# DLR-RM/3DObjectTracking

Measured on NVIDIA H100. Metric: pose-opt iterations/sec (bodies x corr_iters), higher is better.
Workload: dtype f32

## Files before the change

### 3dobjecttracking_b200/csrc/m3t_b200_track2.cuh

```cuda
#pragma once

#include "m3t_b200_kernels.cuh"
#include "m3t_b200_views.cuh"

namespace m3tb {

constexpr int kGroup = 512;
constexpr int kDistBytes = kDistributionLength * kGroup * 4;
constexpr int kClusterStage = 96;
constexpr int kClusterBytes = 2 * kClusterStage * 32;
constexpr int kFixedDynBytes = kDistBytes + kClusterBytes;

struct BinImage {
  const uint16_t* px;
  unsigned pitch;
};

struct Shared2 {
  float pose[12];
  float rb2c[12], db2c[12];
  float dc2b[12];
  float cw2c[12], dw2c[12];
  float view_o[2][4];
  Tile ctile, dtile;
  unsigned long long depth_bar, lut_bar, ctile_bar;
  float red[32][32];
  float a[36], b[6], x[6];
  int views[2][2];
  FrameView cframe, dframe;
  int stamp_n[2];
  BodyDev body;
  CameraDev cams[2];
  ModelDev models[2];
  const float4* info[2];
  BinImage bins;
};

template <int T>
__device__ __forceinline__ void GroupBarrier(int group) {
  if (T == kGroup) __syncthreads();
  else asm volatile("bar.sync %0, %1;" ::"r"(group + 1), "r"(kGroup) : "memory");
}

struct LineRegs {
  float cbx, cby, cbz, cu, cv, nu, nv, dr, ncts, mean, var;
  bool valid;
};

template <int T>
__device__ __forceinline__ void Stamp2(const TrackArgs& args, Shared2& sh) {
  const int tid = threadIdx.x, warp = tid >> 5;
  if (!args.phase_clock || (tid & 31) != 0) return;
  if (warp != T / 32 - 1 && !(T > kGroup && warp == kGroup / 32 - 1)) return;
  const int half = (T > kGroup && tid < kGroup) ? 1 : 0;
  const int i = sh.stamp_n[half];
  if (i < kPhaseSlots / 2) {
    args.phase_clock[size_t(blockIdx.x) * kPhaseSlots + half * (kPhaseSlots / 2) + i] = clock64();
    sh.stamp_n[half] = i + 1;
  }
}

#define M3TB_STAMP_AT(slot, cond)                                                                  \
  do {                                                                                             \
    if (args.phase_clock && (cond)) args.phase_clock[size_t(body_id) * kPhaseSlots + (slot)] = clock64(); \
  } while (0)

template <bool LUT_SMEM, int S>
__device__ __forceinline__ void WalkFast(int scale, int base, float minor_f, float step, int stride_major, int stride_minor,
                                         const uint16_t* tile_px, const float2* __restrict__ lut_g, const float2* lut_s,
                                         const float* __restrict__ lf, const float* __restrict__ lb, bool rev,
                                         float* dist_col) {
  float wf[8], wb[8];
#pragma unroll
  for (int w = 0; w < kLineSegments; ++w) {
    float pf = 1.0f, pb = 1.0f;
    if (S > 0) {
      int idx[S > 0 ? S : 1];
#pragma unroll
      for (int k = 0; k < S; ++k) {
        idx[k] = tile_px[base + int(minor_f) * stride_minor];
        base += stride_major;
        minor_f += step;
      }
      float2 l[S > 0 ? S : 1];
#pragma unroll
      for (int k = 0; k < S; ++k) l[k] = LutFetch<LUT_SMEM>(lut_g, lut_s, idx[k]);
#pragma unroll
      for (int k = 0; k < S; ++k) { pf *= l[k].x; pb *= l[k].y; }
    } else {
#pragma unroll 1
      for (int k = 0; k < scale; ++k) {
        const int idx = tile_px[base + int(minor_f) * stride_minor];
        const float2 l = LutFetch<LUT_SMEM>(lut_g, lut_s, idx);
        pf *= l.x;
        pb *= l.y;
        base += stride_major;
        minor_f += step;
      }
    }
    if (S > 1 || (S == 0 && scale > 1)) {
      if (pf != 0.0f || pb != 0.0f) {
        float sum = pf;
        sum += pb;
        pf /= sum;
        pb /= sum;
      } else {
        pf = 0.5f;
        pb = 0.5f;
      }
    }
    wf[w & 7] = pf;
    wb[w & 7] = pb;
    if (w >= 7) {
      float val = 1.0f;
#pragma unroll
      for (int k = 0; k < kFunctionLength; ++k) {
        const float f = rev ? wf[(w - k) & 7] : wf[(w + 1 + k) & 7];
        const float b = rev ? wb[(w - k) & 7] : wb[(w + 1 + k) & 7];
        val *= f * lf[k] + b * lb[k];
      }
      dist_col[(rev ? kLineSegments - 1 - w : w - 7) * kGroup] = val;
    }
  }
}

template <bool LUT_SMEM>
__device__ __noinline__ void WalkSlow(int scale, int bs, int nb, bool horizontal, int major, float minor_f, float step,
                                      const FrameView& frame, const Tile& tile, const uint16_t* tile_px, const BinImage& bins,
                                      const float2* __restrict__ lut_g, const float2* lut_s, const float* lf,
                                      const float* lb, bool rev, float* dist_col) {
  float sf[kLineSegments], sb[kLineSegments];
#pragma unroll 1
  for (int s = 0; s < kLineSegments; ++s) {
    float pf = 1.0f, pb = 1.0f;
#pragma unroll 1
    for (int k = 0; k < scale; ++k) {
      const int minor = int(minor_f);
      const int x = horizontal ? major : minor, y = horizontal ? minor : major;
      const unsigned tx = unsigned(x - tile.x0), ty = unsigned(y - tile.y0);
      int idx;
      if (tx < unsigned(tile.w) && ty < unsigned(tile.h)) {
        idx = tile_px[ty * unsigned(tile.pitch) + tx];
      } else if (bins.px && x >= frame.x0 && x < frame.x1 && y >= frame.y0 && y < frame.y1) {
        idx = __ldg(reinterpret_cast<const uint16_t*>(reinterpret_cast<const uint8_t*>(bins.px) + size_t(unsigned(y)) * bins.pitch) + x);
      } else {
        const uint8_t* p = FramePtr(frame, x, y, 3u);
        idx = int(LutSlot(unsigned((int(__ldg(p)) >> bs) * nb * nb + (int(__ldg(p + 1)) >> bs) * nb + (int(__ldg(p + 2)) >> bs))));
      }
      const float2 l = LutFetch<LUT_SMEM>(lut_g, lut_s, idx);
      pf *= l.x;
      pb *= l.y;
      ++major;
      minor_f += step;
    }
    sf[s] = pf;
    sb[s] = pb;
  }
  if (scale > 1) {
#pragma unroll 1
    for (int s = 0; s < kLineSegments; ++s) {
      if (sf[s] != 0.0f || sb[s] != 0.0f) {
        float sum = sf[s];
        sum += sb[s];
        sf[s] /= sum;
        sb[s] /= sum;
      } else {
        sf[s] = 0.5f;
        sb[s] = 0.5f;
      }
    }
  }
#pragma unroll 1
  for (int d = 0; d < kDistributionLength; ++d) {
    float val = 1.0f;
#pragma unroll 1
    for (int k = 0; k < kFunctionLength; ++k) {
      const int s = rev ? kLineSegments - 1 - (d + k) : d + k;
      val *= sf[s] * lf[k] + sb[s] * lb[k];
    }
    dist_col[d * kGroup] = val;
  }
}

template <bool LUT_SMEM>
__device__ __forceinline__ void RegionLine2(const RegionIter& it, const RegionParamsDev& rp, const float4 p0, const float4 p1,
                                            const FrameView& frame, const Tile& tile, const uint16_t* tile_px,
                                            const BinImage& bins, const float2* __restrict__ lut_g, const float2* lut_s,
                                            const float* __restrict__ lf, const float* __restrict__ lb,
                                            float* dist_col, LineRegs& L) {
  L.valid = false;
  float x, y, z;
  PoseApply(it.b2c, p0.x, p0.y, p0.z, x, y, z);
  float nu = it.b2c[0] * p0.w + it.b2c[1] * p1.x + it.b2c[2] * p1.y;
  float nv = it.b2c[4] * p0.w + it.b2c[5] * p1.x + it.b2c[6] * p1.y;
  {
    float zz = nu * nu + nv * nv;
    if (zz > 0.0f) { float n = sqrtf(zz); nu /= n; nv /= n; }
  }
  float center_u = x * it.fu / z + it.ppu;
  float center_v = y * it.fv / z + it.ppv;
  L.cbx = p0.x; L.cby = p0.y; L.cbz = p0.z;
  L.cu = center_u; L.cv = center_v; L.nu = nu; L.nv = nv;
  float continuous_distance = fminf(p1.w, p1.z) * it.fu / (z * it.fscale);
  if (continuous_distance < rp.min_continuous_distance) return;
  if (z <= 0.0f) return;
  int icu = int(center_u + 0.5f), icv = int(center_v + 0.5f);
  if (icu < 0 || icu > it.w_m1 || icv < 0 || icv > it.h_m1) return;
  const bool horizontal = fabsf(nv) < fabsf(nu);
  const float c_major = horizontal ? center_u : center_v;
  const float c_minor = horizontal ? center_v : center_u;
  const float n_major = horizontal ? nu : nv;
  const float n_minor = horizontal ? nv : nu;
  const int major_m1 = horizontal ? it.w_m1 : it.h_m1;
  const int minor_m1 = horizontal ? it.h_m1 : it.w_m1;
  const int minor_m2 = horizontal ? it.h_m2 : it.w_m2;
  const float step = n_minor / n_major;
  int major = int(c_major - it.ll_half_m1);
  const int major_end = major + it.ll_m1;
  float minor_f = c_minor + step * (float(major) - c_major) + 0.5f;
  const float minor_f_end = minor_f + step * float(it.ll_m1);
  if (major < 0 || major_end > major_m1 || int(minor_f) < 0 || int(minor_f) > minor_m1 || int(minor_f_end) < 1 ||
      int(minor_f_end) > minor_m2)
    return;
  const bool rev = !(n_major > 0.0f);
  {
    const int mi0 = int(minor_f), mi1 = int(minor_f_end);
    const int minor_lo = min(mi0, mi1) - 1, minor_hi = max(mi0, mi1) + 1;
    const int x_lo = horizontal ? major : minor_lo, x_hi = horizontal ? major_end : minor_hi;
    const int y_lo = horizontal ? minor_lo : major, y_hi = horizontal ? minor_hi : major_end;
    const bool inside = x_lo >= tile.x0 && x_hi < tile.x0 + tile.w && y_lo >= tile.y0 && y_hi < tile.y0 + tile.h;
    if (inside) {
      const int stride_major = horizontal ? 1 : tile.pitch;
      const int stride_minor = horizontal ? tile.pitch : 1;
      const int base = horizontal ? (major - tile.x0) - tile.y0 * tile.pitch : (major - tile.y0) * tile.pitch - tile.x0;
      switch (it.scale) {
        case 1: WalkFast<LUT_SMEM, 1>(1, base, minor_f, step, stride_major, stride_minor, tile_px, lut_g, lut_s, lf, lb, rev, dist_col); break;
        case 2: WalkFast<LUT_SMEM, 2>(2, base, minor_f, step, stride_major, stride_minor, tile_px, lut_g, lut_s, lf, lb, rev, dist_col); break;
        case 4: WalkFast<LUT_SMEM, 4>(4, base, minor_f, step, stride_major, stride_minor, tile_px, lut_g, lut_s, lf, lb, rev, dist_col); break;
        case 6: WalkFast<LUT_SMEM, 6>(6, base, minor_f, step, stride_major, stride_minor, tile_px, lut_g, lut_s, lf, lb, rev, dist_col); break;
        default: WalkFast<LUT_SMEM, 0>(it.scale, base, minor_f, step, stride_major, stride_minor, tile_px, lut_g, lut_s, lf, lb, rev, dist_col); break;
      }
    } else {
      WalkSlow<LUT_SMEM>(it.scale, rp.bitshift, rp.n_bins, horizontal, major, minor_f, step, frame, tile, tile_px, bins,
                         lut_g, lut_s, lf, lb, rev, dist_col);
    }
  }
  L.ncts = fabsf(n_major) / it.fscale;
  L.dr = (roundf(c_major - it.ll_m1_half) + it.ll_m1_half - c_major) / n_major;
  float dist[kDistributionLength];
  float area = 0.0f;
#pragma unroll
  for (int d = 0; d < kDistributionLength; ++d) {
    dist[d] = dist_col[d * kGroup];
    area += dist[d];
  }
#pragma unroll
  for (int d = 0; d < kDistributionLength; ++d) {
    dist[d] /= area;
    dist_col[d * kGroup] = dist[d];
  }
  float mean_from_begin = 0.0f;
#pragma unroll
  for (int d = 0; d < kDistributionLength; ++d) mean_from_begin += float(d) * dist[d];
  float var = 0.0f;
#pragma unroll
  for (int d = 0; d < kDistributionLength; ++d) {
    float dd = float(d) - mean_from_begin;
    var += (dd * dd) * dist[d];
  }
  L.mean = mean_from_begin - (float(kDistributionLength) - 1.0f) / 2.0f;
  L.var = fmaxf(var, rp.min_expected_variance);
  L.valid = true;
}

__device__ __forceinline__ void RegionGradient2(const RegionIter& it, const RegionParamsDev& rp, const LineRegs& L,
                                                const float* dist_col, int opt_iteration, float (&acc)[27]) {
  if (!L.valid) return;
  float x, y, z;
  PoseApply(it.b2c, L.cbx, L.cby, L.cbz, x, y, z);
  float fu_z = it.fu / z, fv_z = it.fv / z;
  float xfu_z = x * fu_z, yfv_z = y * fv_z;
  float delta_cs = (L.nu * (xfu_z + it.ppu - L.cu) + L.nv * (yfv_z + it.ppv - L.cv) - L.dr) * L.ncts;
  float dll;
  if (opt_iteration < rp.n_global_iterations) {
    dll = (L.mean - delta_cs) / L.var;
  } else {
    int upper = int(delta_cs + (float(kDistributionLength) + 1.0f) / 2.0f);
    int lower = upper - 1;
    if (upper <= 0 || upper >= kDistributionLength) return;
    dll = (logf(dist_col[upper * kGroup]) - logf(dist_col[lower * kGroup])) * rp.learning_rate / L.var;
  }
  float dc0 = L.ncts * L.nu * fu_z;
  float dc1 = L.ncts * L.nv * fv_z;
  float dc2 = L.ncts * (-L.nu * xfu_z - L.nv * yfv_z) / z;
  float J[6];
  J[3] = dc0 * it.b2c[0] + dc1 * it.b2c[4] + dc2 * it.b2c[8];
  J[4] = dc0 * it.b2c[1] + dc1 * it.b2c[5] + dc2 * it.b2c[9];
  J[5] = dc0 * it.b2c[2] + dc1 * it.b2c[6] + dc2 * it.b2c[10];
  J[0] = L.cby * J[5] - L.cbz * J[4];
  J[1] = L.cbz * J[3] - L.cbx * J[5];
  J[2] = L.cbx * J[4] - L.cby * J[3];
  float weight = rp.min_expected_variance / (L.ncts * L.ncts * it.variance);
  float wg = weight * dll;
  float wh = weight / L.var;
#pragma unroll
  for (int r = 0; r < 6; ++r) {
    acc[r] += wg * J[r];
#pragma unroll
    for (int c = 0; c <= r; ++c) acc[6 + Tri(r, c)] -= (wh * J[r]) * J[c];
  }
}

__device__ __forceinline__ void TensorCopyG2S(void* dst_smem, const CUtensorMap* map, int x, int y, int z,
                                              unsigned long long* bar) {
  asm volatile(
      "cp.async.bulk.tensor.3d.shared::cluster.global.tile.mbarrier::complete_tx::bytes [%0], [%1, {%2, %3, %4}], [%5];" ::"r"(
          SmemAddr(dst_smem)),
      "l"(reinterpret_cast<unsigned long long>(map)), "r"(x), "r"(y), "r"(z), "r"(SmemAddr(bar))
      : "memory");
}

__device__ __forceinline__ void SnapTile(Tile& t, const FrameView& f, int budget, int max_w = 256) {
  const int vx0 = f.x0, vx1 = f.x1, vy0 = f.y0, vy1 = f.y1;
  if (t.w <= 0 || t.h <= 0 || vx1 - vx0 < 64 || vy1 - vy0 < kTileBoxRows || budget < 64 * kTileBoxRows * 2) {
    t.w = t.h = t.pitch = 0;
    return;
  }
  int w = min(max_w, (max(t.w, 64) + 31) / 32 * 32);
  w = min(w, (vx1 - vx0) / 32 * 32);
  w = max(w, 64);
  if (w > vx1 - vx0) { t.w = t.h = t.pitch = 0; return; }
  int h = (t.h + kTileBoxRows - 1) / kTileBoxRows * kTileBoxRows;
  h = min(h, (vy1 - vy0) / kTileBoxRows * kTileBoxRows);
  while (w * h * 2 > budget) {
    if (h >= w && h > kTileBoxRows) h -= kTileBoxRows;
    else if (w > 64) w -= 32;
    else if (h > kTileBoxRows) h -= kTileBoxRows;
    else { t.w = t.h = t.pitch = 0; return; }
  }
  int x0 = (t.x0 + (t.w - w) / 2) & ~7, y0 = t.y0 + (t.h - h) / 2;
  x0 = max((vx0 + 7) & ~7, min(x0, (vx1 - w) & ~7));
  y0 = max(vy0, min(y0, vy1 - h));
  if (x0 < vx0 || x0 + w > vx1) { t.w = t.h = t.pitch = 0; return; }
  t.x0 = x0; t.y0 = y0; t.w = w; t.h = h; t.pitch = w;
}

__device__ __forceinline__ void PublishPoseProducts(const float (&pose)[12], bool has_color, bool has_depth, bool store_pose,
                                                    Shared2& sh) {
  const bool writer = (threadIdx.x & 31) == 0;
  if (store_pose && writer) {
#pragma unroll
    for (int i = 0; i < 12; ++i) sh.pose[i] = pose[i];
  }
  if (has_color) {
    float w[12], o[12];
#pragma unroll
    for (int i = 0; i < 12; ++i) w[i] = sh.cw2c[i];
    PoseMul(w, pose, o);
    float v0 = 0.0f, v1 = 0.0f, v2 = 0.0f;
    const bool nz = ViewOrientation(o, v0, v1, v2);
    if (writer) {
#pragma unroll
      for (int i = 0; i < 12; ++i) sh.rb2c[i] = o[i];
      sh.view_o[0][0] = v0; sh.view_o[0][1] = v1; sh.view_o[0][2] = v2; sh.view_o[0][3] = nz ? 1.0f : 0.0f;
    }
  }
  if (has_depth) {
    float w[12], o[12], inv[12];
#pragma unroll
    for (int i = 0; i < 12; ++i) w[i] = sh.dw2c[i];
    PoseMul(w, pose, o);
    PoseInverse(o, inv);
    float v0 = 0.0f, v1 = 0.0f, v2 = 0.0f;
    const bool nz = ViewOrientation(o, v0, v1, v2);
    if (writer) {
#pragma unroll
      for (int i = 0; i < 12; ++i) { sh.db2c[i] = o[i]; sh.dc2b[i] = inv[i]; }
      sh.view_o[1][0] = v0; sh.view_o[1][1] = v1; sh.view_o[1][2] = v2; sh.view_o[1][3] = nz ? 1.0f : 0.0f;
    }
  }
}

__device__ __forceinline__ bool SolveAndUpdateSerial(Shared2& sh, bool has_color, bool has_depth) {
  constexpr int n = 6;
  unsigned key[n];
  int pm[n];
#pragma unroll
  for (int i = 0; i < n; ++i) { key[i] = __float_as_uint(fabsf(sh.a[i * (n + 1)])); pm[i] = i; }
#pragma unroll
  for (int k = 0; k < n - 1; ++k) {
    int p = k;
    unsigned big = key[k];
#pragma unroll
    for (int q = k + 1; q < n; ++q)
      if (key[q] > big) { big = key[q]; p = q; }
#pragma unroll
    for (int q = k + 1; q < n; ++q)
      if (p == q) {
        const unsigned tk = key[k]; key[k] = key[q]; key[q] = tk;
        const int tp = pm[k]; pm[k] = pm[q]; pm[q] = tp;
      }
  }
  float A[n][n];
  float dst[n];
#pragma unroll
  for (int i = 0; i < n; ++i) {
#pragma unroll
    for (int j = 0; j <= i; ++j) A[i][j] = sh.a[pm[i] * n + pm[j]];
    dst[i] = sh.b[pm[i]];
  }
  float D[n];
  bool zero_matrix = false;
#pragma unroll
  for (int k = 0; k < n; ++k) {
    if (k > 0) {
      float temp[n];
#pragma unroll
      for (int j = 0; j < k; ++j) temp[j] = D[j] * A[k][j];
#pragma unroll
      for (int i = k; i < n; ++i) {
        float acc = 0.0f;
#pragma unroll
        for (int j = 0; j < k; ++j) acc += A[i][j] * temp[j];
        if (!zero_matrix) A[i][k] -= acc;
      }
    }
    const float akk = A[k][k];
    const bool pivot_is_valid = fabsf(akk) > 0.0f;
    if (k == 0 && !pivot_is_valid) zero_matrix = true;
    D[k] = akk;
    if (!zero_matrix && pivot_is_valid) {
#pragma unroll
      for (int i = k + 1; i < n; ++i) A[i][k] /= akk;
    }
  }
#pragma unroll
  for (int j = 0; j < n; ++j) {
#pragma unroll
    for (int r = j + 1; r < n; ++r) dst[r] -= A[r][j] * dst[j];
  }
  {
    const float tolerance = 1.0f / 3.402823466e+38f;
#pragma unroll
    for (int r = 0; r < n; ++r) {
      if (fabsf(D[r]) > tolerance) dst[r] /= D[r];
      else dst[r] = 0.0f;
    }
  }
#pragma unroll
  for (int j = n - 1; j >= 1; --j) {
#pragma unroll
    for (int r = 0; r < j; ++r) dst[r] -= A[j][r] * dst[j];
  }
  __syncwarp();
#pragma unroll
  for (int r = 0; r < n; ++r) sh.x[pm[r]] = dst[r];
  __syncwarp();
  float theta[n];
  bool nan = false;
#pragma unroll
  for (int i = 0; i < n; ++i) { theta[i] = sh.x[i]; nan = nan || isnan(theta[i]); }
  if (nan) return false;
  float e[9];
  ExpSkew(theta, e);
  float var[12] = {e[0], e[1], e[2], theta[3], e[3], e[4], e[5], theta[4], e[6], e[7], e[8], theta[5]};
  float cur[12], np[12];
#pragma unroll
  for (int i = 0; i < 12; ++i) cur[i] = sh.pose[i];
  PoseMul(cur, var, np);
  __syncwarp();
  PublishPoseProducts(np, has_color, has_depth, true, sh);
  return true;
}

__device__ __forceinline__ unsigned char* DynSmem() {
  extern __shared__ __align__(128) unsigned char dyn[];
  return dyn;
}
template <bool LUT_SMEM>
constexpr unsigned kLutBytes = LUT_SMEM ? unsigned(16 * 16 * 16 * sizeof(float2)) : 0u;
template <bool LUT_SMEM>
__device__ __forceinline__ float* DistCol() {
  unsigned tid;
  asm volatile("mov.u32 %0, %%tid.x;" : "=r"(tid));
  return reinterpret_cast<float*>(DynSmem() + kLutBytes<LUT_SMEM>) + (tid & (kGroup - 1));
}
__device__ __forceinline__ bool DoPhase(const Shared2& sh, const TrackArgs& args, bool region, unsigned phase) {
  return (region ? sh.body.has_region : sh.body.has_depth) && (args.phases & phase);
}

struct Track2Ready {
  bool lut, ctile, depth;
};

template <int T, bool LUT_SMEM, bool POINTS>
__device__ __forceinline__ void LineCorrespondence(const TrackArgs& args, Shared2& sh, int corr, int& view_r, int view_d,
                                                   int& n_lines, LineRegs& L, Track2Ready& ready) {
  const int tid = threadIdx.x, lane = tid & 31, warp = tid >> 5, item = tid & (kGroup - 1);
  const BodyDev& body = sh.body;
  const ModelDev* rmodel = &sh.models[0];
  if (item >= kGroup - 32) {
    const int v = ClosestViewPrunedWarp(sh.info[0], rmodel->sorted_views, rmodel->n_clusters, rmodel->orientations4,
                                        rmodel->n_views, sh.view_o[0], view_r);
    if (lane == 0) sh.views[corr & 1][0] = v;
  }
  if (POINTS && DoPhase(sh, args, false, PH_DEPTH_CORR) && warp == T / 32 - 2) {
    const ModelDev* dmodel = &sh.models[1];
    const int v = ClosestViewPrunedWarp(sh.info[1], dmodel->sorted_views, dmodel->n_clusters, dmodel->orientations4,
                                        dmodel->n_views, sh.view_o[1], view_d);
    if (lane == 0) sh.views[corr & 1][1] = v;
  }
  GroupBarrier<T>(0);
  view_r = sh.views[corr & 1][0];
  Stamp2<T>(args, sh);
  RegionIter rit;
  MakeRegionIter(body.rp, sh.cams[0], sh.rb2c, corr, rit);
  const float4* pts = rmodel->points + size_t(view_r) * rmodel->n_points * 2;
  float4 p0 = make_float4(0.0f, 0.0f, 0.0f, 0.0f), p1 = p0;
  if (item < min(rmodel->n_points, min(args.line_cap, kGroup))) { p0 = __ldg(pts + 2 * item); p1 = __ldg(pts + 2 * item + 1); }
  n_lines = AdaptiveCount(body.rp.n_lines_max, body.rp.use_adaptive_coverage, body.rp.reference_contour_length,
                          body.rp.use_adaptive_coverage ? __ldg(rmodel->view_scalars + view_r) : 0.0f,
                          rmodel->max_view_scalar, rmodel->n_points);
  n_lines = min(n_lines, min(args.line_cap, kGroup));
  const int body_id = blockIdx.x;
  M3TB_STAMP_AT(118, tid == T - 32 && !ready.ctile);
  if (!ready.lut) { MbarWait(&sh.lut_bar, 0); ready.lut = true; }
  if (!ready.ctile) { MbarWait(&sh.ctile_bar, 0); ready.ctile = true; M3TB_STAMP_AT(119, tid == T - 32); }
  L.valid = false;
  if (item < n_lines) {
    const uint16_t* tile_px = reinterpret_cast<const uint16_t*>(DynSmem() + sh.ctile.offset);
    const float2* lut_g = args.lut + size_t(blockIdx.x) * args.lut_stride;
    const float2* lut_s = reinterpret_cast<const float2*>(DynSmem());
    RegionLine2<LUT_SMEM>(rit, body.rp, p0, p1, sh.cframe, sh.ctile, tile_px, sh.bins, lut_g, lut_s, args.lookup_f,
                          args.lookup_b, DistCol<LUT_SMEM>(), L);
  }
  Stamp2<T>(args, sh);
}

template <int T, bool LINES>
__device__ __forceinline__ void PointCorrespondence(const TrackArgs& args, Shared2& sh, int corr, int& view_d, int& n_points,
                                                    PointState& P, Track2Ready& ready) {
  const int tid = threadIdx.x, lane = tid & 31, item = tid & (kGroup - 1);
  const BodyDev& body = sh.body;
  const ModelDev* dmodel = &sh.models[1];
  if (!LINES || !DoPhase(sh, args, true, PH_REGION_CORR)) {
    if (item >= kGroup - 32) {
      const int v = ClosestViewPrunedWarp(sh.info[1], dmodel->sorted_views, dmodel->n_clusters, dmodel->orientations4,
                                          dmodel->n_views, sh.view_o[1], view_d);
      if (lane == 0) sh.views[corr & 1][1] = v;
    }
    GroupBarrier<T>(1);
  }
  view_d = sh.views[corr & 1][1];
  Stamp2<T>(args, sh);
  DepthIter dit;
  MakeDepthIter(body.dp, sh.cams[1], sh.db2c, sh.dc2b, corr, dit);
  const float4* pts = dmodel->points + size_t(view_d) * dmodel->n_points * 2;
  float4 p0 = make_float4(0.0f, 0.0f, 0.0f, 0.0f), p1 = p0;
  if (item < min(dmodel->n_points, min(args.point_cap, kGroup))) { p0 = __ldg(pts + 2 * item); p1 = __ldg(pts + 2 * item + 1); }
  n_points = AdaptiveCount(body.dp.n_points_max, body.dp.use_adaptive_coverage, body.dp.reference_surface_area,
                           body.dp.use_adaptive_coverage ? __ldg(dmodel->view_scalars + view_d) : 0.0f,
                           dmodel->max_view_scalar, dmodel->n_points);
  n_points = min(n_points, min(args.point_cap, kGroup));
  if (!ready.depth) { MbarWait(&sh.depth_bar, 0); ready.depth = true; }
  P.valid = false;
  if (item < n_points) {
    const uint16_t* tile_px = reinterpret_cast<const uint16_t*>(DynSmem() + sh.dtile.offset);
    DepthPoint<false>(dit, body.dp, p0, p1, sh.dframe, sh.dtile, tile_px, P);
  }
  Stamp2<T>(args, sh);
}

template <int HALF>
__device__ __forceinline__ void HalvingLevel(float (&v)[32], int lane) {
  const bool upper = (lane & HALF) != 0;
#pragma unroll
  for (int k = 0; k < HALF; ++k) {
    const float send = upper ? v[k] : v[k + HALF];
    const float keep = upper ? v[k + HALF] : v[k];
    v[k] = keep + __shfl_xor_sync(0xffffffffu, send, HALF);
  }
}
__device__ __forceinline__ float WarpReduce27(const float (&acc)[27]) {
  const int lane = threadIdx.x & 31;
  float v[32];
#pragma unroll
  for (int k = 0; k < 32; ++k) v[k] = k < 27 ? acc[k] : 0.0f;
  HalvingLevel<16>(v, lane);
  HalvingLevel<8>(v, lane);
  HalvingLevel<4>(v, lane);
  HalvingLevel<2>(v, lane);
  HalvingLevel<1>(v, lane);
  return v[0];
}

template <int T, bool POINTS>
__device__ __forceinline__ void SumAndSolve(const TrackArgs& args, Shared2& sh) {
  constexpr int kW = T / 32;
  const int lane = threadIdx.x & 31;
  const int l = lane < 27 ? lane : 26;
  float s4[4] = {0.0f, 0.0f, 0.0f, 0.0f};
#pragma unroll
  for (int w = 0; w < kW; ++w) s4[w & 3] += sh.red[w][l];
  const float v = (s4[0] + s4[1]) + (s4[2] + s4[3]);
  int i, j;
  TriInv(l >= 6 ? l - 6 : 0, i, j);
  float aval = 0.0f - v;
  if (i == j) aval += (i < 3) ? sh.body.tikhonov_rotation : sh.body.tikhonov_translation;
  const bool is_b = l < 6;
  float* p1 = is_b ? &sh.b[l] : &sh.a[i * 6 + j];
  float* p2 = is_b ? &sh.b[l] : &sh.a[j * 6 + i];
  const float val = is_b ? 0.0f + v : aval;
  *p1 = val;
  *p2 = val;
  __syncwarp();
  Stamp2<T>(args, sh);
  SolveAndUpdateSerial(sh, sh.body.has_region != 0, POINTS && sh.body.has_depth);
  Stamp2<T>(args, sh);
}

template <int T, bool LUT_SMEM, bool LINES, bool POINTS>
__device__ __forceinline__ void ItemLoop(const TrackArgs& args, Shared2& sh, Track2Ready& ready) {
  constexpr int kW = T / 32;
  const int tid = threadIdx.x, warp = tid >> 5, item = tid & (kGroup - 1);
  const int body_id = blockIdx.x;
  int* counts = args.counts + 4 * body_id;
  LineRegs L;
  PointState P;
  L.valid = false;
  P.valid = false;
  L.cbx = L.cby = L.cbz = L.cu = L.cv = L.nu = L.nv = L.dr = L.ncts = L.mean = L.var = 0.0f;
  P.cbx = P.cby = P.cbz = P.nx = P.ny = P.nz = P.yx = P.yy = P.yz = 0.0f;
  int n_lines = 0, n_points = 0;
  int view_r = LINES ? counts[2] : 0, view_d = POINTS ? counts[3] : 0;

  for (int corr = args.corr_begin; corr < args.corr_end; ++corr) {
    if (LINES && DoPhase(sh, args, true, PH_REGION_CORR))
      LineCorrespondence<T, LUT_SMEM, POINTS>(args, sh, corr, view_r, view_d, n_lines, L, ready);
    if (POINTS && DoPhase(sh, args, false, PH_DEPTH_CORR)) PointCorrespondence<T, LINES>(args, sh, corr, view_d, n_points, P, ready);

    for (int upd = 0; upd < args.n_update; ++upd) {
      const int opt_iteration = args.opt_base + upd;
      float acc[27];
#pragma unroll
      for (int k = 0; k < 27; ++k) acc[k] = 0.0f;
      if (LINES && DoPhase(sh, args, true, PH_REGION_GH)) {
        RegionIter rit;
        MakeRegionIter(sh.body.rp, sh.cams[0], sh.rb2c, corr, rit);
        RegionGradient2(rit, sh.body.rp, L, DistCol<LUT_SMEM>(), opt_iteration, acc);
      }
      if (POINTS && DoPhase(sh, args, false, PH_DEPTH_GH)) {
        DepthIter dit;
        MakeDepthIter(sh.body.dp, sh.cams[1], sh.db2c, sh.dc2b, corr, dit);
        DepthGradient(dit, P, acc);
      }
      sh.red[warp][tid & 31] = WarpReduce27(acc);
      Stamp2<T>(args, sh);
      __syncthreads();
      Stamp2<T>(args, sh);
      if (LINES && warp == kW - 1) SumAndSolve<T, POINTS>(args, sh);
      __syncthreads();
      if (!LINES && sh.body.has_depth) {
        if (item >= kGroup - 32) {
          float pose[12];
#pragma unroll
          for (int i = 0; i < 12; ++i) pose[i] = sh.pose[i];
          PublishPoseProducts(pose, false, true, false, sh);
        }
        GroupBarrier<T>(1);
      }
      Stamp2<T>(args, sh);
    }
  }

  const BodyDev& body = sh.body;
  if (LINES && (args.phases & PH_STORE_REGION) && body.has_region) {
    const int lcap = args.line_cap;
    float* g_rst = args.region_state + size_t(body_id) * RF_COUNT * lcap;
    if (item < n_lines) {
      const int i = item;
      g_rst[RF_CBX * lcap + i] = L.cbx; g_rst[RF_CBY * lcap + i] = L.cby; g_rst[RF_CBZ * lcap + i] = L.cbz;
      g_rst[RF_CU * lcap + i] = L.cu; g_rst[RF_CV * lcap + i] = L.cv;
      g_rst[RF_NU * lcap + i] = L.nu; g_rst[RF_NV * lcap + i] = L.nv;
      g_rst[RF_VALID * lcap + i] = L.valid ? 1.0f : 0.0f;
      if (L.valid) {
        g_rst[RF_DR * lcap + i] = L.dr; g_rst[RF_NCTS * lcap + i] = L.ncts;
        g_rst[RF_MEAN * lcap + i] = L.mean; g_rst[RF_VAR * lcap + i] = L.var;
#pragma unroll
        for (int d = 0; d < kDistributionLength; ++d) g_rst[(RF_DIST0 + d) * lcap + i] = DistCol<LUT_SMEM>()[d * kGroup];
      }
    }
    if (item == 0) { counts[0] = n_lines; counts[2] = view_r; }
  }
  if (POINTS && (args.phases & PH_STORE_DEPTH) && body.has_depth) {
    const int pcap = args.point_cap;
    float* g_dst = args.depth_state + size_t(body_id) * DF_COUNT * pcap;
    if (item < n_points) {
      const int i = item;
      g_dst[DF_CBX * pcap + i] = P.cbx; g_dst[DF_CBY * pcap + i] = P.cby; g_dst[DF_CBZ * pcap + i] = P.cbz;
      g_dst[DF_NX * pcap + i] = P.nx; g_dst[DF_NY * pcap + i] = P.ny; g_dst[DF_NZ * pcap + i] = P.nz;
      g_dst[DF_VALID * pcap + i] = P.valid ? 1.0f : 0.0f;
      if (P.valid) {
        g_dst[DF_YX * pcap + i] = P.yx; g_dst[DF_YY * pcap + i] = P.yy; g_dst[DF_YZ * pcap + i] = P.yz;
      }
    }
    if (item == 0) { counts[1] = n_points; counts[3] = view_d; }
  }
}

template <int T, bool LUT_SMEM>
__global__ void __launch_bounds__(T, 1) k_track2(const __grid_constant__ TrackArgs args) {
  extern __shared__ __align__(128) unsigned char dyn[];
  __shared__ Shared2 sh;
  constexpr int kW = T / 32;
  const int body_id = blockIdx.x;
  const int tid = threadIdx.x, lane = tid & 31, warp = tid >> 5;
  const BodyDev& gbody = args.bodies[body_id];
  if (!gbody.set) return;
  {
    const int* src = reinterpret_cast<const int*>(&gbody);
    int* dst = reinterpret_cast<int*>(&sh.body);
    for (int k = tid; k < int(sizeof(BodyDev) / 4); k += T) dst[k] = __ldg(src + k);
    if (gbody.has_region) {
      const int* c = reinterpret_cast<const int*>(&args.color_cams[gbody.color_camera]);
      const int* m = reinterpret_cast<const int*>(&args.region_models[gbody.region_model]);
      for (int k = tid; k < int(sizeof(CameraDev) / 4); k += T) reinterpret_cast<int*>(&sh.cams[0])[k] = __ldg(c + k);
      for (int k = tid; k < int(sizeof(ModelDev) / 4); k += T) reinterpret_cast<int*>(&sh.models[0])[k] = __ldg(m + k);
    }
    if (gbody.has_depth) {
      const int* c = reinterpret_cast<const int*>(&args.depth_cams[gbody.depth_camera]);
      const int* m = reinterpret_cast<const int*>(&args.depth_models[gbody.depth_model]);
      for (int k = tid; k < int(sizeof(CameraDev) / 4); k += T) reinterpret_cast<int*>(&sh.cams[1])[k] = __ldg(c + k);
      for (int k = tid; k < int(sizeof(ModelDev) / 4); k += T) reinterpret_cast<int*>(&sh.models[1])[k] = __ldg(m + k);
    }
    if (tid < 2) sh.stamp_n[tid] = 0;
  }
  __syncthreads();
  M3TB_STAMP_AT(120, tid == T - 32);
  const BodyDev& body = sh.body;
  const bool has_region = body.has_region, has_depth = body.has_depth;
  const float2* lut_g = args.lut + size_t(body_id) * args.lut_stride;
  constexpr unsigned lut_bytes = kLutBytes<LUT_SMEM>;
  Stamp2<T>(args, sh);

  const CameraDev* ccam = has_region ? &sh.cams[0] : nullptr;
  const CameraDev* dcam = has_depth ? &sh.cams[1] : nullptr;
  const ModelDev* rmodel = has_region ? &sh.models[0] : nullptr;
  const ModelDev* dmodel = has_depth ? &sh.models[1] : nullptr;
  const bool do_rcorr = has_region && (args.phases & PH_REGION_CORR);
  const bool do_dcorr = has_depth && (args.phases & PH_DEPTH_CORR);
  FrameView cframe, dframe;
  cframe.dev = cframe.host = dframe.dev = dframe.host = nullptr;
  cframe.dev_pitch = cframe.host_pitch = dframe.dev_pitch = dframe.host_pitch = 0u;
  cframe.x0 = cframe.y0 = cframe.x1 = cframe.y1 = dframe.x0 = dframe.y0 = dframe.x1 = dframe.y1 = 0;
  if (ccam) cframe = MakeFrameView(*ccam, args.roi[2 * body_id + 0]);
  if (dcam) dframe = MakeFrameView(*dcam, args.roi[2 * body_id + 1]);
  if (tid < 12) sh.pose[tid] = args.poses[12 * body_id + tid];
  if (tid >= 32 && tid < 44 && ccam) sh.cw2c[tid - 32] = ccam->w2c[tid - 32];
  if (tid >= 64 && tid < 76 && dcam) sh.dw2c[tid - 64] = dcam->w2c[tid - 64];
  float4* cl_smem = reinterpret_cast<float4*>(dyn + lut_bytes + kDistBytes);
  const bool stage_r = do_rcorr && rmodel->n_clusters <= kClusterStage;
  const bool stage_d = do_dcorr && dmodel->n_clusters <= kClusterStage;
  if (stage_r)
    for (int k = tid; k < 2 * rmodel->n_clusters; k += T) cl_smem[k] = __ldg(rmodel->cluster_info + k);
  if (stage_d)
    for (int k = tid; k < 2 * dmodel->n_clusters; k += T) cl_smem[2 * kClusterStage + k] = __ldg(dmodel->cluster_info + k);
  const bool need_lut = LUT_SMEM && do_rcorr;
  const bool tma = args.tma_mode != 0;
  if (tid == 0) {
    if (LUT_SMEM) MbarInit(&sh.lut_bar, 1);
    MbarInit(&sh.depth_bar, 1);
    MbarInit(&sh.ctile_bar, 1);
    sh.cframe = cframe;
    sh.dframe = dframe;
    sh.info[0] = stage_r ? cl_smem : (rmodel ? rmodel->cluster_info : nullptr);
    sh.info[1] = stage_d ? cl_smem + 2 * kClusterStage : (dmodel ? dmodel->cluster_info : nullptr);
    sh.bins.px = (tma && ccam) ? ccam->bins : nullptr;
    sh.bins.pitch = ccam ? ccam->bin_pitch : 0u;
  }
  __syncthreads();
  M3TB_STAMP_AT(121, tid == T - 32);
  if (warp == kW - 1) {
    float pose[12];
#pragma unroll
    for (int i = 0; i < 12; ++i) pose[i] = sh.pose[i];
    PublishPoseProducts(pose, ccam != nullptr, dcam != nullptr, false, sh);
    M3TB_STAMP_AT(122, lane == 0);
  }
  if (need_lut && tid == 0) {
    const unsigned bytes = unsigned(body.rp.n_bins * body.rp.n_bins * body.rp.n_bins) * sizeof(float2);
    MbarExpectTx(&sh.lut_bar, bytes);
    BulkCopyG2S(dyn, lut_g, bytes, &sh.lut_bar);
  }
  if (tma) {
    if (tid == 32 % T) {
      M3TB_STAMP_AT(124, true);
      Tile ct, dt;
      ct.x0 = ct.y0 = ct.w = ct.h = ct.pitch = 0; ct.offset = lut_bytes + kFixedDynBytes;
      dt = ct;
      if (args.tile_bytes > 0) {
        float b2c[12];
        if (do_rcorr) {
          int s_max = 1;
          for (int c = args.corr_begin; c < args.corr_end; ++c) s_max = max(s_max, LastValid(body.rp.scales, body.rp.n_scales, c));
          PoseMul(ccam->w2c, sh.pose, b2c);
          RoiRect(b2c, ccam->fu, ccam->fv, ccam->ppu, ccam->ppv, ccam->width, ccam->height, rmodel->radius,
                  0.5f * float(kLineSegments * s_max) + 2.0f + 12.0f, 1, ct);
        }
        if (do_dcorr) {
          float d_max = 0.0f;
          for (int c = args.corr_begin; c < args.corr_end; ++c)
            d_max = fmaxf(d_max, LastValid(body.dp.considered_distances, body.dp.n_considered_distances, c));
          PoseMul(dcam->w2c, sh.pose, b2c);
          const float z = b2c[11];
          const float reach = (z > 2.0f * dmodel->radius) ? d_max * dcam->fu / (z - dmodel->radius) + 2.0f + 8.0f : 0.0f;
          RoiRect(b2c, dcam->fu, dcam->fv, dcam->ppu, dcam->ppv, dcam->width, dcam->height, dmodel->radius, reach, 1, dt);
        }
        const int budget = args.tile_bytes - 256;
        SnapTile(dt, dframe, budget * 2 / 5, args.tma_max_w);
        const int dbytes = dt.w * dt.h * 2;
        SnapTile(ct, cframe, budget - dbytes, args.tma_max_w);
        dt.offset = lut_bytes + kFixedDynBytes + unsigned(ct.w * ct.h * 2);
      }
      sh.ctile = ct;
      sh.dtile = dt;
      M3TB_STAMP_AT(125, true);
      if (ct.w > 0) {
        const CUtensorMap* map = (args.tma_mode == 2 ? args.tmaps_global : args.bin_maps) + ((ct.w - 64) >> 5);
        MbarExpectTx(&sh.ctile_bar, unsigned(ct.w * ct.h * 2));
#pragma unroll 1
        for (int r = 0; r < ct.h; r += kTileBoxRows)
          TensorCopyG2S(dyn + ct.offset + size_t(r) * ct.w * 2, map, ct.x0, ct.y0 + r, body.color_camera, &sh.ctile_bar);
      }
      if (dt.w > 0) {
        const CUtensorMap* map = (args.tma_mode == 2 ? args.tmaps_global + kTileWidths : args.depth_maps) + ((dt.w - 64) >> 5);
        MbarExpectTx(&sh.depth_bar, unsigned(dt.w * dt.h * 2));
#pragma unroll 1
        for (int r = 0; r < dt.h; r += kTileBoxRows)
          TensorCopyG2S(dyn + dt.offset + size_t(r) * dt.w * 2, map, dt.x0, dt.y0 + r, body.depth_camera, &sh.depth_bar);
      }
      M3TB_STAMP_AT(126, true);
    }
  } else {
    if (tid == 32 % T) {
      Tile ct, dt;
      ct.x0 = ct.y0 = ct.w = ct.h = ct.pitch = 0; ct.offset = lut_bytes + kFixedDynBytes;
      dt = ct;
      if (args.tile_bytes > 0) {
        float b2c[12];
        if (do_rcorr) {
          int s_max = 1;
          for (int c = args.corr_begin; c < args.corr_end; ++c) s_max = max(s_max, LastValid(body.rp.scales, body.rp.n_scales, c));
          PoseMul(ccam->w2c, sh.pose, b2c);
          RoiRect(b2c, ccam->fu, ccam->fv, ccam->ppu, ccam->ppv, ccam->width, ccam->height, rmodel->radius,
                  0.5f * float(kLineSegments * s_max) + 2.0f + 12.0f, 4, ct);
        }
        if (do_dcorr) {
          float d_max = 0.0f;
          for (int c = args.corr_begin; c < args.corr_end; ++c)
            d_max = fmaxf(d_max, LastValid(body.dp.considered_distances, body.dp.n_considered_distances, c));
          PoseMul(dcam->w2c, sh.pose, b2c);
          const float z = b2c[11];
          const float reach = (z > 2.0f * dmodel->radius) ? d_max * dcam->fu / (z - dmodel->radius) + 2.0f + 8.0f : 0.0f;
          RoiRect(b2c, dcam->fu, dcam->fv, dcam->ppu, dcam->ppv, dcam->width, dcam->height, dmodel->radius, reach, 8, dt);
        }
        ClipTile(ct, cframe, 4);
        ClipTile(dt, dframe, 8);
        int budget = args.tile_bytes - 256;
        FitTile(dt, budget * 2 / 5, 8);
        const int dbytes = (dt.w * dt.h * 2 + 127) / 128 * 128;
        FitTile(ct, budget - dbytes, 4);
        const int cbytes = (ct.w * ct.h * 2 + 127) / 128 * 128;
        dt.offset = lut_bytes + kFixedDynBytes + unsigned(cbytes);
      }
      sh.ctile = ct;
      sh.dtile = dt;
    }
  }
  __syncthreads();
  const Tile ctile = sh.ctile, dtile = sh.dtile;
  bool depth_ready = dtile.w <= 0;
  bool ctile_ready = ctile.w <= 0 || !tma;
  if (!tma) {
    if (dtile.w > 0) {
      if (warp == 0) {
        const unsigned row_bytes = unsigned(dtile.w) * 2u;
        if (lane == 0) MbarExpectTx(&sh.depth_bar, row_bytes * unsigned(dtile.h));
        __syncwarp();
        for (int r = lane; r < dtile.h; r += 32)
          BulkCopyG2S(dyn + dtile.offset + size_t(r) * row_bytes,
                      dcam->image + size_t(dtile.y0 + r) * dcam->pitch + size_t(dtile.x0) * 2u, row_bytes, &sh.depth_bar);
      }
    }
    if (ctile.w > 0) {
      const int groups_per_row = ctile.w >> 2;
      const int n_groups = groups_per_row * ctile.h;
      const int bs = body.rp.bitshift, nb = body.rp.n_bins;
      uint2* out = reinterpret_cast<uint2*>(dyn + ctile.offset);
      auto bin = [&](unsigned b, unsigned gch, unsigned rch) {
        return LutSlot(((b >> bs) * unsigned(nb) + (gch >> bs)) * unsigned(nb) + (rch >> bs));
      };
      for (int g0 = tid; g0 < n_groups; g0 += 4 * T) {
        unsigned w[4][3];
  #pragma unroll
        for (int u = 0; u < 4; ++u) {
          const int g = g0 + u * T;
          if (g < n_groups) {
            const int r = g / groups_per_row, c = g - r * groups_per_row;
            const unsigned* src = reinterpret_cast<const unsigned*>(ccam->image + size_t(ctile.y0 + r) * ccam->pitch +
                                                                    size_t(ctile.x0 + 4 * c) * 3u);
            w[u][0] = __ldg(src); w[u][1] = __ldg(src + 1); w[u][2] = __ldg(src + 2);
          }
        }
  #pragma unroll
        for (int u = 0; u < 4; ++u) {
          const int g = g0 + u * T;
          if (g < n_groups) {
            const unsigned w0 = w[u][0], w1 = w[u][1], w2 = w[u][2];
            const unsigned i0 = bin(w0 & 0xffu, (w0 >> 8) & 0xffu, (w0 >> 16) & 0xffu);
            const unsigned i1 = bin(w0 >> 24, w1 & 0xffu, (w1 >> 8) & 0xffu);
            const unsigned i2 = bin((w1 >> 16) & 0xffu, w1 >> 24, w2 & 0xffu);
            const unsigned i3 = bin((w2 >> 8) & 0xffu, (w2 >> 16) & 0xffu, w2 >> 24);
            out[g] = make_uint2(i0 | (i1 << 16), i2 | (i3 << 16));
          }
        }
      }
    }
    __syncthreads();
  }

  Track2Ready ready = {!need_lut, ctile_ready, depth_ready};
  Stamp2<T>(args, sh);

  if (T == kGroup) ItemLoop<T, LUT_SMEM, true, true>(args, sh, ready);
  else if (tid >= kGroup) ItemLoop<T, LUT_SMEM, true, false>(args, sh, ready);
  else ItemLoop<T, LUT_SMEM, false, true>(args, sh, ready);

  if (args.phases & PH_SOLVE)
    if (tid < 12) args.poses[12 * body_id + tid] = sh.pose[tid];
  if (need_lut && !ready.lut) MbarWait(&sh.lut_bar, 0);
  if (!ready.depth) MbarWait(&sh.depth_bar, 0);
  if (!ready.ctile) MbarWait(&sh.ctile_bar, 0);
}

}
```

### 3dobjecttracking_b200/csrc/m3t_b200_views.cuh

```cuda
#pragma once

#include <cuda_runtime.h>
#include <stdint.h>

#include <algorithm>
#include <cmath>
#include <cstring>
#include <vector>

namespace m3tb {

constexpr int kViewClusterSize = 32;
constexpr int kMaxViewClusterSlots = 8;

struct ViewClustersHost {
  std::vector<float> info;
  std::vector<float> sorted;
  int n_clusters = 0;
};

inline float FloatUp(double v) {
  float f = float(v);
  if (double(f) < v) f = std::nextafterf(f, INFINITY);
  return f;
}
inline float FloatDown(double v) {
  float f = float(v);
  if (double(f) > v) f = std::nextafterf(f, -INFINITY);
  return f;
}

inline void BuildViewClusters(const float* ori, int n, ViewClustersHost& out) {
  out.info.clear();
  out.sorted.assign(size_t(n) * 4, 0.0f);
  out.n_clusters = 0;
  std::vector<int> idx(n);
  for (int i = 0; i < n; ++i) idx[i] = i;
  struct Range { int lo, hi; };
  std::vector<Range> stack, leaves;
  stack.push_back({0, n});
  while (!stack.empty()) {
    const Range r = stack.back();
    stack.pop_back();
    const int cnt = r.hi - r.lo;
    if (cnt <= kViewClusterSize) {
      if (cnt > 0) leaves.push_back(r);
      continue;
    }
    float mn[3] = {INFINITY, INFINITY, INFINITY}, mx[3] = {-INFINITY, -INFINITY, -INFINITY};
    for (int i = r.lo; i < r.hi; ++i)
      for (int a = 0; a < 3; ++a) {
        const float v = ori[3 * idx[i] + a];
        mn[a] = std::min(mn[a], v);
        mx[a] = std::max(mx[a], v);
      }
    int axis = 0;
    for (int a = 1; a < 3; ++a)
      if (mx[a] - mn[a] > mx[axis] - mn[axis]) axis = a;
    int left = ((cnt / 2 + kViewClusterSize - 1) / kViewClusterSize) * kViewClusterSize;
    if (left >= cnt) left = cnt / 2;
    std::sort(idx.begin() + r.lo, idx.begin() + r.hi, [&](int p, int q) {
      const float vp = ori[3 * p + axis], vq = ori[3 * q + axis];
      return vp < vq || (vp == vq && p < q);
    });
    stack.push_back({r.lo + left, r.hi});
    stack.push_back({r.lo, r.lo + left});
  }
  std::sort(leaves.begin(), leaves.end(), [](const Range& p, const Range& q) { return p.lo < q.lo; });
  out.n_clusters = int(leaves.size());
  out.info.assign(size_t(out.n_clusters) * 8, 0.0f);
  for (int c = 0; c < out.n_clusters; ++c) {
    const Range r = leaves[c];
    std::sort(idx.begin() + r.lo, idx.begin() + r.hi);
    double m[3] = {0.0, 0.0, 0.0};
    for (int i = r.lo; i < r.hi; ++i) {
      const float* v = ori + 3 * idx[i];
      const double nv = std::sqrt(double(v[0]) * v[0] + double(v[1]) * v[1] + double(v[2]) * v[2]);
      if (nv > 0.0)
        for (int a = 0; a < 3; ++a) m[a] += v[a] / nv;
    }
    double nm = std::sqrt(m[0] * m[0] + m[1] * m[1] + m[2] * m[2]);
    if (!(nm > 1e-12)) { m[0] = 0.0; m[1] = 0.0; m[2] = 1.0; nm = 1.0; }
    float cf[3] = {float(m[0] / nm), float(m[1] / nm), float(m[2] / nm)};
    const double cn = std::sqrt(double(cf[0]) * cf[0] + double(cf[1]) * cf[1] + double(cf[2]) * cf[2]);
    double vc_max = -INFINITY, vc_min = INFINITY, vperp_max = 0.0, vnorm_max = 0.0;
    for (int i = r.lo; i < r.hi; ++i) {
      const float* v = ori + 3 * idx[i];
      const double vc = (double(v[0]) * cf[0] + double(v[1]) * cf[1] + double(v[2]) * cf[2]) / (cn * cn);
      double perp2 = 0.0, n2 = 0.0;
      for (int a = 0; a < 3; ++a) {
        const double d = double(v[a]) - vc * cf[a];
        perp2 += d * d;
        n2 += double(v[a]) * v[a];
      }
      vc_max = std::max(vc_max, vc);
      vc_min = std::min(vc_min, vc);
      vperp_max = std::max(vperp_max, std::sqrt(perp2));
      vnorm_max = std::max(vnorm_max, std::sqrt(n2));
      float* s = out.sorted.data() + size_t(i) * 4;
      s[0] = v[0]; s[1] = v[1]; s[2] = v[2];
      const int32_t orig = idx[i];
      std::memcpy(&s[3], &orig, 4);
    }
    float* f = out.info.data() + size_t(c) * 8;
    f[0] = cf[0]; f[1] = cf[1]; f[2] = cf[2];
    f[3] = FloatUp(vc_max);
    f[4] = FloatDown(vc_min);
    f[5] = FloatUp(vperp_max * (1.0 + 1e-6));
    f[6] = FloatUp(2e-5 * std::max(vnorm_max, 1e-30));
    const uint32_t packed = uint32_t(r.lo) | (uint32_t(r.hi - r.lo) << 24);
    std::memcpy(&f[7], &packed, 4);
  }
}

__host__ __device__ inline float ViewClusterBound(float cx, float cy, float cz, float vc_max, float vc_min, float vperp_max,
                                                  float slack_scale, float o0, float o1, float o2, float on2, float onorm) {
  const float p = o0 * cx + o1 * cy + o2 * cz;
  const float along = fmaxf(p * vc_max, p * vc_min);
  const float perp = sqrtf(fmaxf(on2 - p * p, 0.0f) + 1e-6f * on2);
  return along + perp * vperp_max + slack_scale * onorm;
}

inline int ClosestViewPrunedHost(const ViewClustersHost& vc, const float* ori, int n_views, const float o[3], int prev,
                                 int* n_evaluated) {
  const float on2 = o[0] * o[0] + o[1] * o[1] + o[2] * o[2];
  const float onorm = std::sqrt(on2);
  prev = std::min(std::max(prev, 0), n_views - 1);
  const float lb = o[0] * ori[3 * prev] + o[1] * ori[3 * prev + 1] + o[2] * ori[3 * prev + 2];
  float best = -1.0f;
  int idx = 0x7fffffff, evaluated = 0;
  for (int c = 0; c < vc.n_clusters; ++c) {
    const float* f = vc.info.data() + size_t(c) * 8;
    const float ub = ViewClusterBound(f[0], f[1], f[2], f[3], f[4], f[5], f[6], o[0], o[1], o[2], on2, onorm);
    if (ub < lb) continue;
    uint32_t packed;
    std::memcpy(&packed, &f[7], 4);
    const int first = int(packed & 0xffffffu), cnt = int(packed >> 24);
    for (int k = 0; k < cnt; ++k) {
      const float* s = vc.sorted.data() + size_t(first + k) * 4;
      const float dot = o[0] * s[0] + o[1] * s[1] + o[2] * s[2];
      int32_t vi;
      std::memcpy(&vi, &s[3], 4);
      if (dot > best || (dot == best && vi < idx)) { best = dot; idx = vi; }
      ++evaluated;
    }
  }
  if (n_evaluated) *n_evaluated = evaluated;
  return idx == 0x7fffffff ? 0 : idx;
}

#ifdef __CUDACC__
__device__ __forceinline__ int ClosestViewPrunedWarp(const float4* info, const float4* __restrict__ sorted,
                                                     int n_clusters, const float4* __restrict__ ori4, int n_views,
                                                     const float* vo, int prev) {
  constexpr unsigned kFull = 0xffffffffu;
  const int lane = threadIdx.x & 31;
  const float o0 = vo[0], o1 = vo[1], o2 = vo[2];
  if (vo[3] == 0.0f || n_views <= 0) return 0;
  const float on2 = o0 * o0 + o1 * o1 + o2 * o2;
  const float onorm = sqrtf(on2);
  prev = min(max(prev, 0), n_views - 1);
  const float4 qp = __ldg(ori4 + prev);
  const float lb = o0 * qp.x + o1 * qp.y + o2 * qp.z;
  float best = -1.0f;
  int idx = 0x7fffffff;
  for (int c0 = 0; c0 < n_clusters; c0 += 64) {
    float4 ia[2], ib[2];
#pragma unroll
    for (int h = 0; h < 2; ++h) {
      const int c = c0 + 32 * h + lane;
      if (c < n_clusters) { ia[h] = info[2 * c]; ib[h] = info[2 * c + 1]; }
      else { ia[h] = make_float4(0.0f, 0.0f, 0.0f, 0.0f); ib[h] = ia[h]; }
    }
#pragma unroll
    for (int h = 0; h < 2; ++h) {
      const int c = c0 + 32 * h + lane;
      bool cand = false;
      if (c < n_clusters) {
        const float ub = ViewClusterBound(ia[h].x, ia[h].y, ia[h].z, ia[h].w, ib[h].x, ib[h].y, ib[h].z, o0, o1, o2, on2, onorm);
        cand = !(ub < lb);
      }
      const unsigned packed = __float_as_uint(ib[h].w);
      unsigned m = __ballot_sync(kFull, cand);
      while (m) {
        unsigned pk[4];
#pragma unroll
        for (int u = 0; u < 4; ++u) {
          const int j = m ? __ffs(m) - 1 : 0;
          const unsigned v = __shfl_sync(kFull, packed, j);
          pk[u] = m ? v : 0u;
          m &= m - 1u;
        }
        float4 q[4];
#pragma unroll
        for (int u = 0; u < 4; ++u) {
          const int first = int(pk[u] & 0xffffffu), cnt = int(pk[u] >> 24);
          q[u] = lane < cnt ? __ldg(sorted + first + lane) : make_float4(0.0f, 0.0f, 0.0f, 0.0f);
        }
#pragma unroll
        for (int u = 0; u < 4; ++u) {
          const int cnt = int(pk[u] >> 24);
          const float dot = o0 * q[u].x + o1 * q[u].y + o2 * q[u].z;
          const int vi = __float_as_int(q[u].w);
          if (lane < cnt && (dot > best || (dot == best && vi < idx))) { best = dot; idx = vi; }
        }
      }
    }
  }
  unsigned key = __float_as_uint(best);
  key = (key & 0x80000000u) ? ~key : (key | 0x80000000u);
  const unsigned kmax = __reduce_max_sync(kFull, key);
  const unsigned candi = key == kmax ? unsigned(idx) : 0x7fffffffu;
  const int ri = int(__reduce_min_sync(kFull, candi));
  const unsigned minus_one = ~__float_as_uint(-1.0f);
  return (ri == 0x7fffffff || kmax <= minus_one) ? 0 : ri;
}
#endif

}
```

Before: 4.392 million.

## Spread closest-view search across all warps of the group

```diff
diff --git a/3dobjecttracking_b200/csrc/m3t_b200_track2.cuh b/3dobjecttracking_b200/csrc/m3t_b200_track2.cuh
--- a/3dobjecttracking_b200/csrc/m3t_b200_track2.cuh
+++ b/3dobjecttracking_b200/csrc/m3t_b200_track2.cuh
@@ -26,7 +26,7 @@
   unsigned long long depth_bar, lut_bar, ctile_bar;
   float red[32][32];
   float a[36], b[6], x[6];
-  int views[2][2];
+  uint2 view_slots[2][2][kGroup / 32];
   FrameView cframe, dframe;
   int stamp_n[2];
   BodyDev body;
@@ -493,25 +493,23 @@
   bool lut, ctile, depth;
 };
 
+template <int T>
+__device__ __forceinline__ int GroupClosestView(const TrackArgs& args, Shared2& sh, int corr, int m, int view) {
+  const ModelDev& model = sh.models[m];
+  const int prev = corr > args.corr_begin ? ClosestViewOfSlots<kGroup>(sh.view_slots[(corr - 1) & 1][m]) : view;
+  return ClosestViewPrunedGroup<kGroup>(sh.info[m], model.sorted_views, model.n_clusters, model.orientations4,
+                                        model.n_views, sh.view_o[m], prev, sh.view_slots[corr & 1][m],
+                                        [m] { GroupBarrier<T>(m); });
+}
+
 template <int T, bool LUT_SMEM, bool POINTS>
-__device__ __forceinline__ void LineCorrespondence(const TrackArgs& args, Shared2& sh, int corr, int& view_r, int view_d,
+__device__ __forceinline__ void LineCorrespondence(const TrackArgs& args, Shared2& sh, int corr, int& view_r, int& view_d,
                                                    int& n_lines, LineRegs& L, Track2Ready& ready) {
-  const int tid = threadIdx.x, lane = tid & 31, warp = tid >> 5, item = tid & (kGroup - 1);
+  const int tid = threadIdx.x, item = tid & (kGroup - 1);
   const BodyDev& body = sh.body;
   const ModelDev* rmodel = &sh.models[0];
-  if (item >= kGroup - 32) {
-    const int v = ClosestViewPrunedWarp(sh.info[0], rmodel->sorted_views, rmodel->n_clusters, rmodel->orientations4,
-                                        rmodel->n_views, sh.view_o[0], view_r);
-    if (lane == 0) sh.views[corr & 1][0] = v;
-  }
-  if (POINTS && DoPhase(sh, args, false, PH_DEPTH_CORR) && warp == T / 32 - 2) {
-    const ModelDev* dmodel = &sh.models[1];
-    const int v = ClosestViewPrunedWarp(sh.info[1], dmodel->sorted_views, dmodel->n_clusters, dmodel->orientations4,
-                                        dmodel->n_views, sh.view_o[1], view_d);
-    if (lane == 0) sh.views[corr & 1][1] = v;
-  }
-  GroupBarrier<T>(0);
-  view_r = sh.views[corr & 1][0];
+  view_r = GroupClosestView<T>(args, sh, corr, 0, view_r);
+  if (POINTS && DoPhase(sh, args, false, PH_DEPTH_CORR)) view_d = GroupClosestView<T>(args, sh, corr, 1, view_d);
   Stamp2<T>(args, sh);
   RegionIter rit;
   MakeRegionIter(body.rp, sh.cams[0], sh.rb2c, corr, rit);
@@ -540,18 +538,10 @@
 template <int T, bool LINES>
 __device__ __forceinline__ void PointCorrespondence(const TrackArgs& args, Shared2& sh, int corr, int& view_d, int& n_points,
                                                     PointState& P, Track2Ready& ready) {
-  const int tid = threadIdx.x, lane = tid & 31, item = tid & (kGroup - 1);
+  const int tid = threadIdx.x, item = tid & (kGroup - 1);
   const BodyDev& body = sh.body;
   const ModelDev* dmodel = &sh.models[1];
-  if (!LINES || !DoPhase(sh, args, true, PH_REGION_CORR)) {
-    if (item >= kGroup - 32) {
-      const int v = ClosestViewPrunedWarp(sh.info[1], dmodel->sorted_views, dmodel->n_clusters, dmodel->orientations4,
-                                          dmodel->n_views, sh.view_o[1], view_d);
-      if (lane == 0) sh.views[corr & 1][1] = v;
-    }
-    GroupBarrier<T>(1);
-  }
-  view_d = sh.views[corr & 1][1];
+  if (!LINES || !DoPhase(sh, args, true, PH_REGION_CORR)) view_d = GroupClosestView<T>(args, sh, corr, 1, view_d);
   Stamp2<T>(args, sh);
   DepthIter dit;
   MakeDepthIter(body.dp, sh.cams[1], sh.db2c, sh.dc2b, corr, dit);
diff --git a/3dobjecttracking_b200/csrc/m3t_b200_views.cuh b/3dobjecttracking_b200/csrc/m3t_b200_views.cuh
--- a/3dobjecttracking_b200/csrc/m3t_b200_views.cuh
+++ b/3dobjecttracking_b200/csrc/m3t_b200_views.cuh
@@ -150,6 +150,52 @@
 }
 
 #ifdef __CUDACC__
+template <int B>
+__device__ __forceinline__ void EvaluateViewCandidates(unsigned m, unsigned packed, const float4* __restrict__ sorted,
+                                                       float o0, float o1, float o2, float& best, int& idx) {
+  constexpr unsigned kFull = 0xffffffffu;
+  const int lane = threadIdx.x & 31;
+  while (m) {
+    unsigned pk[B];
+#pragma unroll
+    for (int u = 0; u < B; ++u) {
+      const int j = m ? __ffs(m) - 1 : 0;
+      const unsigned v = __shfl_sync(kFull, packed, j);
+      pk[u] = m ? v : 0u;
+      m &= m - 1u;
+    }
+    float4 q[B];
+#pragma unroll
+    for (int u = 0; u < B; ++u) {
+      const int first = int(pk[u] & 0xffffffu), cnt = int(pk[u] >> 24);
+      q[u] = lane < cnt ? __ldg(sorted + first + lane) : make_float4(0.0f, 0.0f, 0.0f, 0.0f);
+    }
+#pragma unroll
+    for (int u = 0; u < B; ++u) {
+      const int cnt = int(pk[u] >> 24);
+      const float dot = o0 * q[u].x + o1 * q[u].y + o2 * q[u].z;
+      const int vi = __float_as_int(q[u].w);
+      if (lane < cnt && (dot > best || (dot == best && vi < idx))) { best = dot; idx = vi; }
+    }
+  }
+}
+
+__device__ __forceinline__ unsigned ViewKey(float v) {
+  const unsigned k = __float_as_uint(v == 0.0f ? 0.0f : v);
+  return (k & 0x80000000u) ? ~k : (k | 0x80000000u);
+}
+
+__device__ __forceinline__ void WarpViewArgMax(unsigned& key, int& idx) {
+  constexpr unsigned kFull = 0xffffffffu;
+  const unsigned kmax = __reduce_max_sync(kFull, key);
+  idx = int(__reduce_min_sync(kFull, key == kmax ? unsigned(idx) : 0x7fffffffu));
+  key = kmax;
+}
+
+__device__ __forceinline__ int ClosestViewResult(unsigned kmax, int ri) {
+  return (ri == 0x7fffffff || kmax <= ViewKey(-1.0f)) ? 0 : ri;
+}
+
 __device__ __forceinline__ int ClosestViewPrunedWarp(const float4* info, const float4* __restrict__ sorted,
                                                      int n_clusters, const float4* __restrict__ ori4, int n_views,
                                                      const float* vo, int prev) {
@@ -180,40 +226,58 @@
         const float ub = ViewClusterBound(ia[h].x, ia[h].y, ia[h].z, ia[h].w, ib[h].x, ib[h].y, ib[h].z, o0, o1, o2, on2, onorm);
         cand = !(ub < lb);
       }
-      const unsigned packed = __float_as_uint(ib[h].w);
-      unsigned m = __ballot_sync(kFull, cand);
-      while (m) {
-        unsigned pk[4];
-#pragma unroll
-        for (int u = 0; u < 4; ++u) {
-          const int j = m ? __ffs(m) - 1 : 0;
-          const unsigned v = __shfl_sync(kFull, packed, j);
-          pk[u] = m ? v : 0u;
-          m &= m - 1u;
-        }
-        float4 q[4];
-#pragma unroll
-        for (int u = 0; u < 4; ++u) {
-          const int first = int(pk[u] & 0xffffffu), cnt = int(pk[u] >> 24);
-          q[u] = lane < cnt ? __ldg(sorted + first + lane) : make_float4(0.0f, 0.0f, 0.0f, 0.0f);
-        }
-#pragma unroll
-        for (int u = 0; u < 4; ++u) {
-          const int cnt = int(pk[u] >> 24);
-          const float dot = o0 * q[u].x + o1 * q[u].y + o2 * q[u].z;
-          const int vi = __float_as_int(q[u].w);
-          if (lane < cnt && (dot > best || (dot == best && vi < idx))) { best = dot; idx = vi; }
-        }
-      }
-    }
-  }
-  unsigned key = __float_as_uint(best);
-  key = (key & 0x80000000u) ? ~key : (key | 0x80000000u);
-  const unsigned kmax = __reduce_max_sync(kFull, key);
-  const unsigned candi = key == kmax ? unsigned(idx) : 0x7fffffffu;
-  const int ri = int(__reduce_min_sync(kFull, candi));
-  const unsigned minus_one = ~__float_as_uint(-1.0f);
-  return (ri == 0x7fffffff || kmax <= minus_one) ? 0 : ri;
+      EvaluateViewCandidates<4>(__ballot_sync(kFull, cand), __float_as_uint(ib[h].w), sorted, o0, o1, o2, best, idx);
+    }
+  }
+  unsigned key = ViewKey(best);
+  WarpViewArgMax(key, idx);
+  return ClosestViewResult(key, idx);
+}
+
+template <int G>
+__device__ __forceinline__ int ClosestViewOfSlots(const uint2* slots) {
+  const int lane = threadIdx.x & 31;
+  const uint2 s = lane < G / 32 ? slots[lane] : make_uint2(0u, 0x7fffffffu);
+  unsigned key = s.x;
+  int idx = int(s.y);
+  WarpViewArgMax(key, idx);
+  return ClosestViewResult(key, idx);
+}
+
+template <int G, class Barrier>
+__device__ __forceinline__ int ClosestViewPrunedGroup(const float4* info, const float4* __restrict__ sorted,
+                                                      int n_clusters, const float4* __restrict__ ori4, int n_views,
+                                                      const float* vo, int prev, uint2* slots, Barrier barrier) {
+  constexpr unsigned kFull = 0xffffffffu;
+  constexpr int kWarps = G / 32;
+  static_assert(kWarps <= 32 && (G & (G - 1)) == 0, "one slot per warp, read by one warp");
+  const int lane = threadIdx.x & 31, warp = (threadIdx.x & (G - 1)) >> 5;
+  const bool search = vo[3] != 0.0f && n_views > 0;
+  prev = min(max(prev, 0), n_views - 1);
+  const float4 qp = search ? __ldg(ori4 + prev) : make_float4(0.0f, 0.0f, 0.0f, 0.0f);
+  int c = lane * kWarps + warp;
+  float4 ia = make_float4(0.0f, 0.0f, 0.0f, 0.0f), ib = ia;
+  if (search && c < n_clusters) { ia = info[2 * c]; ib = info[2 * c + 1]; }
+  const float o0 = vo[0], o1 = vo[1], o2 = vo[2];
+  const float on2 = o0 * o0 + o1 * o1 + o2 * o2;
+  const float onorm = sqrtf(on2);
+  float best = -1.0f;
+  int idx = 0x7fffffff;
+  for (int c0 = 0; search && c0 < n_clusters; c0 += G, c += G) {
+    bool cand = false;
+    if (c < n_clusters) {
+      const float ub = ViewClusterBound(ia.x, ia.y, ia.z, ia.w, ib.x, ib.y, ib.z, o0, o1, o2, on2, onorm);
+      const float lb = o0 * qp.x + o1 * qp.y + o2 * qp.z;
+      cand = !(ub < lb);
+    }
+    EvaluateViewCandidates<1>(__ballot_sync(kFull, cand), __float_as_uint(ib.w), sorted, o0, o1, o2, best, idx);
+    if (c + G < n_clusters) { ia = info[2 * (c + G)]; ib = info[2 * (c + G) + 1]; }
+  }
+  unsigned key = ViewKey(best);
+  WarpViewArgMax(key, idx);
+  if (lane == 0) slots[warp] = make_uint2(key, unsigned(idx));
+  barrier();
+  return ClosestViewOfSlots<G>(slots);
 }
 #endif
 
```

Measured after the change: 4.561 million, median of 6. 1.04x the previous value.
